# WeiZhang1988/YDORBSLAM

Measured on AMD Instinct MI355X. Metric: ORB extract+match Mkeypoints/sec, higher is better.
Workload: dtype u8

## Files before the change

ydorbslam_amd/csrc/extract_kernels.hip.h:

```cpp
#pragma once
#include <hip/hip_runtime.h>
#include <stdint.h>

#include "quadtree_core.h"
#include "quadtree_flat.h"

#pragma clang fp contract(off)

namespace ydorb {

constexpr int kPad = 19;
constexpr int kBorder = 16;
constexpr int kMaxLevels = 8;
constexpr int kTileMax = 72;
#ifndef QT_THREADS
#define QT_THREADS 512
#endif
constexpr int kQtThreads = QT_THREADS;

struct LevelDev {
  int w, h, pitch;
  int padOff;
  int blurOff, blurPitch;
  int cellBegin, nCells;
  int quota;
  int candOff;
  int kpOff;
  int tabOff;
  int nodeTabOff;
  float scale;
  float size;
};
struct PlanDev {
  int nLevels, nCellsTotal, cellCap, sumQuota;
  int maxX[16];
  unsigned nodeTabFrameStride;
  int blurTileBegin[kMaxLevels + 1];
  int borderBegin[kMaxLevels + 1];
  LevelDev lv[kMaxLevels];
};
#ifndef BLUR_TH
#define BLUR_TH 58
#endif
constexpr int kBlurTW = 64, kBlurTH = BLUR_TH;
struct CellDev {
  short level, x0, y0, x1, y1, pad0;
  int srcOff;
};

__device__ __forceinline__ int reflect101(int i, int n) {
  if (n == 1) return 0;
  while (i < 0 || i >= n) i = i < 0 ? -i : 2 * (n - 1) - i;
  return i;
}

typedef uint32_t __attribute__((aligned(1))) u32_unaligned;
typedef unsigned long long __attribute__((aligned(1))) u64_unaligned;

#ifndef PYR_ROWS
#define PYR_ROWS 8
#endif
constexpr int kPyrRows = PYR_ROWS;
__global__ __launch_bounds__(256) void k_pyr_level0(const uint8_t* __restrict__ img, int stride, size_t frameStride,
                                                    uint8_t* __restrict__ pyr, size_t pyrFrameStride, LevelDev L) {
  const int wx = blockIdx.x * 64 + (threadIdx.x & 63);
  const int yb = (blockIdx.y * 4 + __builtin_amdgcn_readfirstlane(threadIdx.x >> 6)) * kPyrRows;
  const int x0 = wx * 4 - kPad;
  if (x0 + 3 < 0 || x0 >= L.w) return;
  const uint8_t* src = img + (size_t)blockIdx.z * frameStride;
  uint8_t* dst = pyr + (size_t)blockIdx.z * pyrFrameStride + L.padOff + (size_t)kPad * L.pitch + wx * 4;
  const int xa = L.w >= 4 ? min(max(x0, 0), L.w - 4) : 0, sh = 8 * (x0 - xa);
  uint32_t v[kPyrRows];
// ... 294 lines not shown
    return;
  }
  {
    constexpr int COLS = PITCH == 48 ? 8 : 16, ROWS = 64 / COLS, NR = 6;
    const uint8_t* sub = pyr + (size_t)f * pyrFrameStride + c.srcOff;
    const int wpr = (tw + 7) >> 3, ty0 = lane / COLS, wd = lane % COLS;
    const bool colOk = wd < wpr;
    for (int tyb = 0; tyb < th; tyb += ROWS * NR) {
      unsigned long long r[NR];
#pragma unroll
      for (int k = 0; k < NR; k++) {
        const int ty = tyb + ty0 + ROWS * k;
        r[k] = (colOk && ty < th) ? *reinterpret_cast<const u64_unaligned*>(sub + (unsigned)(ty * pitch + 8 * wd)) : 0ull;
      }
#pragma unroll
      for (int k = 0; k < NR; k++) {
        const int ty = tyb + ty0 + ROWS * k;
        if (colOk && ty < th) *reinterpret_cast<unsigned long long*>(tile + ty * PITCH + 8 * wd) = r[k];
      }
    }
  }
  const int sw = bw + 2, sh = bh + 2;
  for (int i = lane; i < (sw * sh + 3) >> 2; i += 64) reinterpret_cast<uint32_t*>(score)[i] = 0;
  __builtin_amdgcn_wave_barrier();
  int n1 = 0;
  {
    const bool wide = bw > 32;
    const int bxl = wide ? lane : (lane & 31), byl = wide ? 0 : (lane >> 5), rowsPerIt = wide ? 1 : 2;
    const uint8_t* p = tile + (byl + 3) * PITCH + bxl + 3;
    unsigned ent = (unsigned)(byl << 6) | (unsigned)bxl;
    const uint16_t t16 = (uint16_t)thr;
    auto step = [&](uint16_t vmask) {
      const uint16_t v = p[0], a = p[3 * PITCH], b = p[-3 * PITCH], cc = p[3], d = p[-3];
      const uint16_t lo1 = min(a, b), hi1 = max(a, b), lo2 = min(cc, d), hi2 = max(cc, d);
      const uint16_t mx = max(lo1, lo2), mn = min(hi1, hi2);
      const uint16_t second = max(mx, mn), third = min(mn, mx);
      const uint16_t s1 = (uint16_t)((uint16_t)(v + t16) - second);
      const uint16_t s2 = (uint16_t)(third - (uint16_t)(v - t16));
      const bool keep = (int16_t)((uint16_t)(s1 | s2) & vmask) < 0;
      const unsigned long long m = __builtin_amdgcn_ballot_w64(keep);
      if (keep) list[n1 + wave_rank(m)] = (uint16_t)(ent | (s1 & 0x8000u) | ((s2 & 0x8000u) >> 1));
      n1 += __popcll(m);
      p += rowsPerIt * PITCH;
      ent += rowsPerIt * 64;
    };
    const bool colOk = bxl < bw;
    unsigned vmA = colOk ? 0xFFFFu : 0x7FFFu, vmF = colOk && byl == 0 ? 0xFFFFu : 0x7FFFu;
    asm volatile("" : "+v"(vmA), "+v"(vmF));
    const uint16_t vmAll = (uint16_t)vmA, vmFirst = (uint16_t)vmF;
    int by0 = 0;
    for (; by0 + rowsPerIt <= bh; by0 += rowsPerIt) step(vmAll);
    if (by0 < bh) step(vmFirst);
  }
  __builtin_amdgcn_wave_barrier();
  int n2 = 0;
  for (int base = 0; base < n1; base += 64) {
    const int j = base + lane;
    bool keep = false;
    unsigned ent = 0;
    if (j < n1) {
      ent = list[j];
      const int by = (ent >> 6) & 127, bx = ent & 63;
      const uint8_t* p = tile + (by + 3) * PITCH + bx + 3;
      const short v = (short)p[0];
      const bool dark = (ent & 0x4000u) != 0;
      const s16x2 sg = dark ? s16x2{1, 1} : s16x2{-1, -1};
      const s16x2 vs = s16x2{v, v} * sg, ng = -sg;
      s16x2 Pd[8];
      Pd[0] = s16x2{(short)p[3 * PITCH], (short)p[-3 * PITCH]} * ng + vs;
      Pd[1] = s16x2{(short)p[3 * PITCH + 1], (short)p[-3 * PITCH - 1]} * ng + vs;
      Pd[2] = s16x2{(short)p[2 * PITCH + 2], (short)p[-2 * PITCH - 2]} * ng + vs;
      Pd[3] = s16x2{(short)p[PITCH + 3], (short)p[-PITCH - 3]} * ng + vs;
      Pd[4] = s16x2{(short)p[3], (short)p[-3]} * ng + vs;
      Pd[5] = s16x2{(short)p[-PITCH + 3], (short)p[PITCH - 3]} * ng + vs;
      Pd[6] = s16x2{(short)p[-2 * PITCH + 2], (short)p[2 * PITCH - 2]} * ng + vs;
      Pd[7] = s16x2{(short)p[-3 * PITCH + 1], (short)p[3 * PITCH - 1]} * ng + vs;
      int best = fast_arc_best(Pd);
      if (__builtin_amdgcn_ballot_w64((ent & 0xC000u) == 0xC000u)) {
        if ((ent & 0xC000u) == 0xC000u) {
          s16x2 Nd[8];
#pragma unroll
          for (int k = 0; k < 8; k++) Nd[k] = -Pd[k];
          best = max(best, fast_arc_best(Nd));
        }
      }
      keep = best > thr;
      if (keep) score[(by + 1) * sw + bx + 1] = (uint8_t)(best - 1);
    }
    const unsigned long long m = __builtin_amdgcn_ballot_w64(keep);
    if (keep) list[n2 + wave_rank(m)] = (uint16_t)ent;
    n2 += __popcll(m);
  }
  __builtin_amdgcn_wave_barrier();
  int n3 = 0;
  uint32_t* dst = cellCand + slot * P.cellCap;
  for (int base = 0; base < n2; base += 64) {
    const int j = base + lane;
    bool keep = false;
    uint32_t rec = 0;
    if (j < n2) {
      const unsigned ent = list[j];
      const int by = (ent >> 6) & 127, bx = ent & 63;
      const uint8_t* q = &score[(by + 1) * sw + bx + 1];
      const uint16_t s = q[0];
      const uint16_t nb = max(max(max((uint16_t)q[-1], (uint16_t)q[1]), max((uint16_t)q[-sw - 1], (uint16_t)q[-sw])),
                              max(max((uint16_t)q[-sw + 1], (uint16_t)q[sw - 1]), max((uint16_t)q[sw], (uint16_t)q[sw + 1])));
      keep = s > nb;
      rec = qt_pack(c.x0 + 3 + bx - kBorder, c.y0 + 3 + by - kBorder, s);
    }
    const unsigned long long m = __builtin_amdgcn_ballot_w64(keep);
    const int pos = n3 + wave_rank(m);
    if (keep && pos < P.cellCap) dst[pos] = rec;
    n3 += __popcll(m);
  }
  if (lane == 0) cellCount[slot] = (uint32_t)min(n3, P.cellCap);
}


struct QtBlockCtx {
  unsigned* w32;
  unsigned long long* w64;
// ... 675 lines not shown
  const int ty = tileId / tilesX, tx = tileId - ty * tilesX;
  const int x0 = tx * TW, y0 = ty * TH;
  const uint8_t* padded = pyr + (size_t)f * pyrFrameStride + L.padOff;
  {
    const int r0 = threadIdx.x / SWW, wd = threadIdx.x - r0 * SWW;
    const int pcol = x0 + 16 + 4 * wd;
    const bool colOk = pcol < L.pitch;
    if (r0 < 14)
#pragma unroll
      for (int r = r0; r < SH; r += 14) {
        const int prow = min(y0 + r + kPad - 3, L.h + 2 * kPad - 1);
        src[r * SWW + wd] = colOk ? *reinterpret_cast<const uint32_t*>(padded + (size_t)prow * L.pitch + pcol) : 0u;
      }
  }
  __syncthreads();
  for (int task = threadIdx.x; task < (SH / 2) * (TW / 4); task += 256) {
    const int rp = task >> 4, g = task & 15;
    uint32_t o[2][4];
#pragma unroll
    for (int h = 0; h < 2; h++) {
      const int r = 2 * rp + h;
      const uint32_t w0 = src[r * SWW + g], w1 = src[r * SWW + g + 1], w2 = src[r * SWW + g + 2];
#pragma unroll
      for (int k = 0; k < 4; k++) {
        const uint32_t lo4 = k ? __builtin_amdgcn_alignbyte(w1, w0, k) : w0, hi4 = k ? __builtin_amdgcn_alignbyte(w2, w1, k) : w1;
        o[h][k] = __builtin_amdgcn_udot4(hi4, 0x00122230u, __builtin_amdgcn_udot4(lo4, 0x38302212u, 0u, false), false);
      }
    }
    *reinterpret_cast<uint4*>(&hb[rp * TW + g * 4]) =
        make_uint4(o[0][0] | (o[1][0] << 16), o[0][1] | (o[1][1] << 16), o[0][2] | (o[1][2] << 16), o[0][3] | (o[1][3] << 16));
  }
  __syncthreads();
  const int c4 = (threadIdx.x & 15) * 4;
#pragma unroll
  for (int r = threadIdx.x >> 4; r < TH; r += 16) {
    const int gy = y0 + r;
    if (!(gy < L.h && x0 + c4 < L.blurPitch)) continue;
    typedef unsigned short u16x2 __attribute__((ext_vector_type(2)));
    const bool odd = r & 1;
    const u16x2 k0 = odd ? u16x2{0, 18} : u16x2{18, 34}, k1 = odd ? u16x2{34, 48} : u16x2{48, 56};
    const u16x2 k2 = odd ? u16x2{56, 48} : u16x2{48, 34}, k3 = odd ? u16x2{34, 18} : u16x2{18, 0};
    const uint32_t* hp = &hb[(r >> 1) * TW + c4];
    const uint4 p0 = *reinterpret_cast<const uint4*>(hp), p1 = *reinterpret_cast<const uint4*>(hp + TW);
    const uint4 p2 = *reinterpret_cast<const uint4*>(hp + 2 * TW), p3 = *reinterpret_cast<const uint4*>(hp + 3 * TW);
    const uint32_t q0[4] = {p0.x, p0.y, p0.z, p0.w}, q1[4] = {p1.x, p1.y, p1.z, p1.w}, q2[4] = {p2.x, p2.y, p2.z, p2.w}, q3[4] = {p3.x, p3.y, p3.z, p3.w};
    uint32_t acc[4];
#pragma unroll
    for (int k = 0; k < 4; k++) {
      acc[k] = __builtin_amdgcn_udot2(__builtin_bit_cast(u16x2, q0[k]), k0, 32768u, false);
      acc[k] = __builtin_amdgcn_udot2(__builtin_bit_cast(u16x2, q1[k]), k1, acc[k], false);
      acc[k] = __builtin_amdgcn_udot2(__builtin_bit_cast(u16x2, q2[k]), k2, acc[k], false);
      acc[k] = __builtin_amdgcn_udot2(__builtin_bit_cast(u16x2, q3[k]), k3, acc[k], false);
    }
    const uint32_t out = (acc[0] >> 16) | ((acc[1] >> 16) << 8) | ((acc[2] >> 16) << 16) | ((acc[3] >> 16) << 24);
    *reinterpret_cast<uint32_t*>(blur + (size_t)f * blurFrameStride + L.blurOff + (size_t)gy * L.blurPitch + x0 + c4) = out;
  }
}

__device__ __forceinline__ float fast_atan2_deg(float y, float x) {
  const float p1 = 0.9997878412794807f * (float)(180 / 3.14159265358979323846);
  const float p3 = -0.3258083974640975f * (float)(180 / 3.14159265358979323846);
  const float p5 = 0.1555786518463281f * (float)(180 / 3.14159265358979323846);
  const float p7 = -0.04432655554792128f * (float)(180 / 3.14159265358979323846);
  const float eps = (float)2.2204460492503131e-16;
  const float ax = fabsf(x), ay = fabsf(y);
  float a, c, c2;
  if (ax >= ay) {
    c = __fdiv_rn(ay, __fadd_rn(ax, eps));
    c2 = __fmul_rn(c, c);
    a = __fmul_rn(__fadd_rn(__fmul_rn(__fadd_rn(__fmul_rn(__fadd_rn(__fmul_rn(p7, c2), p5), c2), p3), c2), p1), c);
  } else {
    c = __fdiv_rn(ax, __fadd_rn(ay, eps));
    c2 = __fmul_rn(c, c);
    a = __fsub_rn(90.f, __fmul_rn(__fadd_rn(__fmul_rn(__fadd_rn(__fmul_rn(__fadd_rn(__fmul_rn(p7, c2), p5), c2), p3), c2), p1), c));
// ... 107 lines not shown
  constexpr int kBias = 24;
  const uint8_t* bl = blur + (size_t)f * blurFrameStride + L.blurOff + (ptrdiff_t)(ky - kBias) * L.blurPitch + (kx - kBias);
  unsigned long long words[4];
#pragma unroll
  for (int t = 0; t < 4; t++) {
    const float4 pt = pat[t];
    const int r0 = __float2int_rn(__fadd_rn(__fmul_rn(pt.x, sinB), __fmul_rn(pt.y, cosA)));
    const int c0 = __float2int_rn(__fsub_rn(__fmul_rn(pt.x, cosA), __fmul_rn(pt.y, sinB)));
    const int r1 = __float2int_rn(__fadd_rn(__fmul_rn(pt.z, sinB), __fmul_rn(pt.w, cosA)));
    const int c1 = __float2int_rn(__fsub_rn(__fmul_rn(pt.z, cosA), __fmul_rn(pt.w, sinB)));
    const int t0 = bl[(unsigned)((r0 + kBias) * L.blurPitch + c0 + kBias)], t1 = bl[(unsigned)((r1 + kBias) * L.blurPitch + c1 + kBias)];
    words[t] = __ballot(t0 < t1);
  }
  if (lane < 4) {
    unsigned long long w = lane == 0 ? words[0] : lane == 1 ? words[1] : lane == 2 ? words[2] : words[3];
    reinterpret_cast<unsigned long long*>(desc + ((size_t)f * cap + outIdx) * 32)[lane] = w;
  }
  if (lane == 0) {
    YdKeyPointDev kp;
    kp.x = (float)kx;
    kp.y = (float)ky;
    if (level) { kp.x = __fmul_rn(kp.x, L.scale); kp.y = __fmul_rn(kp.y, L.scale); }
    kp.size = L.size;
    kp.angle = angle;
    kp.response = (float)qt_r(pk);
    kp.octave = level;
    kp.class_id = -1;
    kps[(size_t)f * cap + outIdx] = kp;
    lvlAngle[(size_t)f * P.sumQuota + slot] = angle;
  }
}


template <int KPW>
__global__ __launch_bounds__(256) void k_orient_describe_n(const uint8_t* __restrict__ pyr, size_t pyrFrameStride,
                                                           const uint8_t* __restrict__ blur, size_t blurFrameStride, PlanDev P,
                                                           const uint32_t* __restrict__ lvlKp, const int* __restrict__ lvlCount,
                                                           YdKeyPointDev* __restrict__ kps, uint8_t* __restrict__ desc, int cap,
                                                           int* __restrict__ nOut, float* __restrict__ lvlAngle) {
  const int lane = threadIdx.x & 63;
  int bx = blockIdx.x, f = blockIdx.y;
  if ((f | 7) < (int)gridDim.y) {
    bx = (f & 7) * (gridDim.x >> 3) + (blockIdx.x >> 3);
    f = (f & ~7) | (blockIdx.x & 7);
  }
  const int slot0 = (bx * 4 + __builtin_amdgcn_readfirstlane(threadIdx.x >> 6)) * KPW;
  if (slot0 >= P.sumQuota) return;
  float4 pat[4];
#pragma unroll
  for (int t = 0; t < 4; t++) pat[t] = reinterpret_cast<const float4*>(kPatternDev)[t * 64 + lane];
  int cnt[kMaxLevels], tot = 0;
#pragma unroll
  for (int l = 0; l < kMaxLevels; l++) { cnt[l] = l < P.nLevels ? lvlCount[f * kMaxLevels + l] : 0; tot += cnt[l]; }
  int level[KPW], outIdx[KPW];
  uint32_t pk[KPW];
  bool valid[KPW];
#pragma unroll
  for (int j = 0; j < KPW; j++) {
    const int slot = min(slot0 + j, P.sumQuota - 1);
    level[j] = 0;
#pragma unroll
    for (int l = 1; l < kMaxLevels; l++)
      if (l < P.nLevels && slot >= P.lv[l].kpOff) level[j] = l;
    pk[j] = __builtin_amdgcn_readfirstlane(lvlKp[(size_t)f * P.sumQuota + slot]);
  }
  if (slot0 == 0 && lane == 0) nOut[f] = min(tot, cap);
  bool any = false;
#pragma unroll
  for (int j = 0; j < KPW; j++) {
    int before = 0, mine = 0;
#pragma unroll
    for (int l = 0; l < kMaxLevels; l++) {
      if (l < level[j]) before += cnt[l];
      if (l == level[j]) mine = cnt[l];
    }
    const int k = slot0 + j - P.lv[level[j]].kpOff;
    outIdx[j] = before + k;
    valid[j] = slot0 + j < P.sumQuota && k < mine && outIdx[j] < cap;
    any = any || valid[j];
  }
  if (!any) return;
  int firstValid = 0;
#pragma unroll
  for (int j = KPW - 1; j >= 0; j--) if (valid[j]) firstValid = j;
#pragma unroll
  for (int j = 0; j < KPW; j++)
    if (!valid[j]) {
#pragma unroll
      for (int i = 0; i < KPW; i++) if (i == firstValid) { pk[j] = pk[i]; level[j] = level[i]; }
    }
  int kx[KPW], ky[KPW], pitch[KPW];
  const uint8_t* org[KPW];
#pragma unroll
  for (int j = 0; j < KPW; j++) {
    const LevelDev& L = P.lv[level[j]];
    kx[j] = qt_x(pk[j]) + kBorder; ky[j] = qt_y(pk[j]) + kBorder;
    pitch[j] = L.pitch;
    const uint8_t* roi = pyr + (size_t)f * pyrFrameStride + L.padOff + (size_t)kPad * L.pitch + kPad;
    org[j] = roi + (ptrdiff_t)(ky[j] - 15) * L.pitch + (kx[j] - 32);
  }
  const int u = lane - 32;
  unsigned narrow = 0;
#pragma unroll
  for (int v = 1; v <= 15; v++) narrow |= (unsigned)(P.maxX[v] == 0) << v;
  int m10[KPW], m01[KPW];
#pragma unroll
  for (int j = 0; j < KPW; j++) {
    m10[j] = 0; m01[j] = 0;
    if (u >= -15 && u <= 15) m10[j] = u * org[j][(unsigned)(15 * pitch[j] + lane)];
    if (lane >= 1 && lane <= 15 && ((narrow >> lane) & 1u)) {
      const int pos = org[j][(unsigned)((15 + lane) * pitch[j] + 32)], neg = org[j][(unsigned)((15 - lane) * pitch[j] + 32)];
      m01[j] = lane * (pos - neg);
    }
  }
#pragma unroll
  for (int v = 1; v <= 15; v++) {
    const int d = P.maxX[v];
    if (d > 0 && u >= -d && u <= d) {
#pragma unroll
      for (int j = 0; j < KPW; j++) {
        const int pos = org[j][(unsigned)((15 + v) * pitch[j] + lane)], neg = org[j][(unsigned)((15 - v) * pitch[j] + lane)];
        m01[j] += v * (pos - neg);
        m10[j] += u * (pos + neg);
      }
    }
  }
#pragma unroll
  for (int o = 32; o >= 1; o >>= 1) {
#pragma unroll
    for (int j = 0; j < KPW; j++) {
      m10[j] += __shfl_xor(m10[j], o, 64);
      m01[j] += __shfl_xor(m01[j], o, 64);
    }
  }
  constexpr int kBias = 24;
  float angle[KPW];
  int tA[KPW][4], tB[KPW][4];
#pragma unroll
  for (int j = 0; j < KPW; j++) {
    const LevelDev& L = P.lv[level[j]];
    angle[j] = fast_atan2_deg((float)m01[j], (float)m10[j]);
    const float rad = __fmul_rn(angle[j], (float)(3.14159265358979323846 / 180.0));
    float sinB, cosA;
    sincos_det(rad, &sinB, &cosA);
    const uint8_t* bl = blur + (size_t)f * blurFrameStride + L.blurOff + (ptrdiff_t)(ky[j] - kBias) * L.blurPitch + (kx[j] - kBias);
#pragma unroll
    for (int t = 0; t < 4; t++) {
      const float4 pt = pat[t];
      const int r0 = __float2int_rn(__fadd_rn(__fmul_rn(pt.x, sinB), __fmul_rn(pt.y, cosA)));
      const int c0 = __float2int_rn(__fsub_rn(__fmul_rn(pt.x, cosA), __fmul_rn(pt.y, sinB)));
      const int r1 = __float2int_rn(__fadd_rn(__fmul_rn(pt.z, sinB), __fmul_rn(pt.w, cosA)));
      const int c1 = __float2int_rn(__fsub_rn(__fmul_rn(pt.z, cosA), __fmul_rn(pt.w, sinB)));
      tA[j][t] = bl[(unsigned)((r0 + kBias) * L.blurPitch + c0 + kBias)];
      tB[j][t] = bl[(unsigned)((r1 + kBias) * L.blurPitch + c1 + kBias)];
    }
  }
#pragma unroll
  for (int j = 0; j < KPW; j++) {
    unsigned long long words[4];
#pragma unroll
    for (int t = 0; t < 4; t++) words[t] = __ballot(tA[j][t] < tB[j][t]);
    if (!valid[j]) continue;
    const LevelDev& L = P.lv[level[j]];
    if (lane < 4) {
      unsigned long long w = lane == 0 ? words[0] : lane == 1 ? words[1] : lane == 2 ? words[2] : words[3];
      reinterpret_cast<unsigned long long*>(desc + ((size_t)f * cap + outIdx[j]) * 32)[lane] = w;
    }
    if (lane == 0) {
      YdKeyPointDev kp;
      kp.x = (float)kx[j];
      kp.y = (float)ky[j];
      if (level[j]) { kp.x = __fmul_rn(kp.x, L.scale); kp.y = __fmul_rn(kp.y, L.scale); }
      kp.size = L.size;
      kp.angle = angle[j];
      kp.response = (float)qt_r(pk[j]);
      kp.octave = level[j];
      kp.class_id = -1;
      kps[(size_t)f * cap + outIdx[j]] = kp;
      lvlAngle[(size_t)f * P.sumQuota + slot0 + j] = angle[j];
    }
  }
}

}
```

ydorbslam_amd/csrc/orb_extractor.hip:

```cpp
#include <hip/hip_runtime.h>
#include <cstdlib>

#include <algorithm>
#include <cmath>
#include <cstdarg>
#include <cstdio>
#include <cstring>
#include <string>
#include <vector>

#include "../../include/ydorb/c_api.h"
#include "extract_kernels.hip.h"
#include "host_buffers.h"
#include "ydorb_host.h"

using namespace ydorb;

namespace {

inline int cvRoundF(float v) { return (int)lrintf(v); }
inline int cvFloorF(float v) { int i = (int)v; return i - (i > v); }
inline int alignUp(int v, int a) { return (v + a - 1) / a * a; }
inline size_t alignUpZ(size_t v, size_t a) { return (v + a - 1) / a * a; }

// ... 20 lines not shown
enum Stage { ST_PYR = 0, ST_FAST, ST_QT, ST_BLUR, ST_DESC, ST_COUNT };
const char* kStageNames[ST_COUNT] = {"pyramid", "fast_cells", "blur", "quadtree_after_blur", "orient_describe"};

}

struct ydorb_extractor {
  YdExtractorConfig cfg{};
  std::vector<float> sf, isf, sf2, isf2;
  std::vector<int> perLevel;
  int maxX[16]{};
  int sumQuota = 0;
  hipStream_t stream = nullptr;
  hipStream_t qtStream[kMaxLevels]{};
  hipEvent_t evFork = nullptr, evJoin[kMaxLevels]{};
  hipEvent_t evFast[kMaxLevels]{};
  int descKpw = 2;
  bool qtInline = false;
  int fastGroups = 1;
  HostPlan plan;
  bool planValid = false;
  int batchCap = 0;
  uint8_t *d_img = nullptr, *d_pyr = nullptr, *d_blur = nullptr;
  uint32_t *d_cellCount = nullptr, *d_cellCand = nullptr, *d_qtCand = nullptr, *d_qtKeys = nullptr, *d_lvlKp = nullptr;
  uint16_t* d_qtNode = nullptr;
  uint8_t* d_nodeScratch = nullptr;
  uint8_t* d_needPass = nullptr;
  int* d_passList = nullptr;
  int *d_lvlCount = nullptr, *d_status = nullptr, *d_nOut = nullptr;
  uint8_t* h_pyr = nullptr;
  size_t h_pyrBytes = 0;
  hipStream_t lastStream = nullptr;
  int *d_lvlMaxN = nullptr, *h_lvlMaxN = nullptr;
  float* d_lvlAngle = nullptr;
  CellDev* d_cells = nullptr;
  int* d_tabInt = nullptr;
  short* d_tabShort = nullptr;
  PyrPadEntry* d_padTab = nullptr;
  PyrColEntry* d_colTab = nullptr;
  int2* d_rowTab = nullptr;
  bool noFusedPads = false;
  YdKeyPointDev* d_kps = nullptr;
  uint8_t* d_desc = nullptr;
  size_t imgBytes = 0;
  uint8_t* h_img = nullptr;
  YdKeyPoint* h_kps = nullptr;
  uint8_t* h_desc = nullptr;
  int* h_nOut = nullptr;
  int* h_status = nullptr;
  int lastFrames = 0;
  bool profiling = false;
  bool profPending = false;
  bool forcePassQuadtree = false;
  hipEvent_t ev[ST_COUNT + 1]{};
  double stageMs[ST_COUNT]{};
  int stageCalls = 0;
};

namespace {

void freeBuffers(ydorb_extractor* e) {
  auto F = [](auto*& p) { if (p) { (void)hipFree(p); p = nullptr; } };
  F(e->d_img); F(e->d_pyr); F(e->d_blur); F(e->d_cellCount); F(e->d_cellCand); F(e->d_qtCand); F(e->d_qtKeys);
  F(e->d_lvlKp); F(e->d_qtNode); F(e->d_needPass); F(e->d_passList); F(e->d_nodeScratch); F(e->d_lvlCount); F(e->d_lvlMaxN); F(e->d_status); F(e->d_nOut); F(e->d_lvlAngle); F(e->d_cells);
  F(e->d_tabInt); F(e->d_tabShort); F(e->d_padTab); F(e->d_colTab); F(e->d_rowTab); F(e->d_kps); F(e->d_desc);
  auto H = [](auto*& p) { if (p) { (void)hipHostFree(p); p = nullptr; } };
  H(e->h_img); H(e->h_kps); H(e->h_desc); H(e->h_nOut); H(e->h_status); H(e->h_lvlMaxN); H(e->h_pyr);
  e->h_pyrBytes = 0;
  e->planValid = false;
}


static int qfItemsFor(long want) { return want <= 8L * kQfThreads ? 8 : want <= 16L * kQfThreads ? 16 : 32; }

void buildFusedLevel(HostPlan& P, int l) {
  const PlanDev& D = P.dev;
  const LevelDev& L = D.lv[l];
  HostPlan::FusedLevel& F = P.fused[l];
  F.on = false;
  if (L.w < 20 || L.h < 20) return;
  const int nd = (L.w + 2 * kPad + 3) >> 2;
  auto srcOf = [&](int p) { return p < kPad ? 2 * kPad - p : p < kPad + L.w ? -1 : p < L.w + 2 * kPad ? 2 * L.w + 2 * kPad - 2 - p : -2; };
  int shift = -1;
  for (int sft = 0; sft < 64 && shift < 0; sft++) {
    bool ok = true;
    for (int c = 0; c < nd && ok; c++)
      for (int j = 0; j < 4; j++) {
        const int sp = srcOf(4 * c + j);
        if (sp >= 0 && ((sp >> 2) + sft) >> 6 != (c + sft) >> 6) ok = false;
      }
    if (ok) shift = sft;
  }
  if (shift < 0) return;
  std::vector<PyrColEntry> col;
  if (l > 0) {
    const LevelDev& Lp = D.lv[l - 1];
    const int* xofs = P.tabInt.data() + P.tab[l].xofs;
// ... 21 lines not shown
      if (dA < 0 || d == dA) dA = d;
      else dB = d;
    }
    PyrPadEntry pe{};
    pe.laneA4 = 4u * (unsigned)(((dA < 0 ? c : dA) + shift) & 63);
    pe.laneB4 = 4u * (unsigned)(((dB < 0 ? c : dB) + shift) & 63);
    pe.selM = 0; pe.selF = 0;
    for (int j = 0; j < 4; j++) {
      const int sp = srcOf(4 * c + j);
      uint32_t m = 0x0c, f;
      if (sp == -1) f = (uint32_t)j;
      else if (sp == -2) f = 0x0c;
      else { m = (uint32_t)(sp & 3) + ((sp >> 2) == dA ? 4u : 0u); f = 4u + (uint32_t)j; }
      pe.selM |= m << (8 * j);
      pe.selF |= f << (8 * j);
    }
    P.padTab.push_back(pe);
  }
  if (l > 0) {
    F.colOff = (int)P.colTab.size();
    P.colTab.insert(P.colTab.end(), col.begin(), col.end());
    F.rowOff = (int)P.rowTab.size();
    const int* yofs = P.tabInt.data() + P.tab[l].yofs;
    const short* beta = P.tabShort.data() + P.tab[l].beta;
    const int rows = alignUp(L.h, 4 * kPyrRowsF);
    for (int y = 0; y < rows; y++) {
      const int dy = std::min(y, L.h - 1);
      P.rowTab.push_back(make_int2(yofs[dy], (int)((uint32_t)(uint16_t)beta[2 * dy] | ((uint32_t)(uint16_t)beta[2 * dy + 1] << 16))));
    }
  }
  F.on = true;
}

int buildPlan(ydorb_extractor* e, int w, int h, HostPlan& P) {
  P = HostPlan();
  P.w = w; P.h = h;
  PlanDev& D = P.dev;
  D.nLevels = e->cfg.n_levels;
  for (int v = 0; v < 16; v++) D.maxX[v] = e->maxX[v];
  size_t padOff = 0, blurOff = 0;
  int kpOff = 0, candOff = 0, maxCellDim = 0;
  for (int l = 0; l < D.nLevels; l++) {
    LevelDev& L = D.lv[l];
    L.w = cvRoundF((float)w * e->isf[l]);
    L.h = cvRoundF((float)h * e->isf[l]);
    if (L.w < 1 || L.h < 1 || L.w > 4000 || L.h > 4000) {
      set_error("level %d size %dx%d out of the supported range (1..4000)", l, L.w, L.h);
      return YDORB_ERR_UNSUPPORTED;
    }
    L.pitch = alignUp(L.w + 2 * kPad, 64);
    L.padOff = (int)padOff;
    padOff += alignUpZ((size_t)(L.h + 2 * kPad) * L.pitch, 256);
    L.blurPitch = alignUp(L.w, 64);
    L.blurOff = (int)blurOff;
    blurOff += alignUpZ((size_t)L.h * L.blurPitch, 256);
    L.quota = e->perLevel[l];
    L.kpOff = kpOff;
    kpOff += L.quota;
    L.scale = e->sf[l];
    L.size = (float)(int)(31 * e->sf[l]);
    L.cellBegin = (int)P.cells.size();
    const int minB = kBorder, maxBX = L.w - kBorder, maxBY = L.h - kBorder;
    const float width = (float)(maxBX - minB), height = (float)(maxBY - minB);
    const int colsNum = (int)(width / 30.0f), rowsNum = (int)(height / 30.0f);
    if (colsNum > 0 && rowsNum > 0) {
      const int cellW = (int)ceilf(width / colsNum), cellH = (int)ceilf(height / rowsNum);
      maxCellDim = std::max(maxCellDim, std::max(cellW, cellH));
      P.levelCellDim[l] = std::max(cellW, cellH);
      for (int i = 0; i < rowsNum; i++) {
        const float iniY = (float)(minB + i * cellH);
        float maxY = iniY + cellH + 6;
        if (iniY >= maxBY - 3) continue;
        if (maxY > maxBY) maxY = (float)maxBY;
        for (int j = 0; j < colsNum; j++) {
          const float iniX = (float)(minB + j * cellW);
          float maxX = iniX + cellW + 6;
          if (iniX >= maxBX - 6) continue;
          if (maxX > maxBX) maxX = (float)maxBX;
          CellDev c{};
          c.level = (short)l;
          c.x0 = (short)iniX; c.y0 = (short)iniY; c.x1 = (short)maxX; c.y1 = (short)maxY;
          c.srcOff = L.padOff + (kPad + c.y0) * L.pitch + kPad + c.x0;
          P.cells.push_back(c);
        }
      }
    }
// ... 77 lines not shown
  }
  P.qtPassLds = std::max<size_t>(P.qtPassLds, 1024);
  return YDORB_OK;
}

int ensurePlan(ydorb_extractor* e, int w, int h, int nFrames) {
  if (e->planValid && e->plan.w == w && e->plan.h == h && nFrames <= e->batchCap) return YDORB_OK;
  HIPCHK(hipStreamSynchronize(e->stream));
  HostPlan P;
  int rc = buildPlan(e, w, h, P);
  if (rc) return rc;
  freeBuffers(e);
  const int B = std::max(nFrames, std::max(1, e->cfg.max_batch));
  e->plan = P;
  e->batchCap = B;
  e->imgBytes = (size_t)w * h;
  const PlanDev& D = P.dev;
  HIPCHK(hipMalloc(&e->d_img, e->imgBytes * B));
  HIPCHK(hipMalloc(&e->d_pyr, P.pyrFrameStride * B));
  HIPCHK(hipMemsetAsync(e->d_pyr, 0, P.pyrFrameStride * B, e->stream));
  HIPCHK(hipMalloc(&e->d_blur, P.blurFrameStride * B));
  HIPCHK(hipMalloc(&e->d_cellCount, sizeof(uint32_t) * D.nCellsTotal * B));
  HIPCHK(hipMalloc(&e->d_cellCand, sizeof(uint32_t) * (size_t)D.nCellsTotal * D.cellCap * B));
  HIPCHK(hipMalloc(&e->d_qtCand, sizeof(uint32_t) * 2 * P.qtFrameStride * B));
  HIPCHK(hipMalloc(&e->d_qtNode, sizeof(uint16_t) * 2 * P.qtFrameStride * B));
  if (D.nodeTabFrameStride) HIPCHK(hipMalloc(&e->d_nodeScratch, (size_t)D.nodeTabFrameStride * B));
  HIPCHK(hipMalloc(&e->d_needPass, (size_t)kMaxLevels * B));
  HIPCHK(hipMemsetAsync(e->d_needPass, 0, (size_t)kMaxLevels * B, e->stream));
  HIPCHK(hipMalloc(&e->d_passList, sizeof(int) * ((size_t)kMaxLevels * B + 1)));
  HIPCHK(hipMemsetAsync(e->d_passList, 0, sizeof(int), e->stream));

  HIPCHK(hipMalloc(&e->d_lvlKp, sizeof(uint32_t) * (size_t)D.sumQuota * B));
  HIPCHK(hipMalloc(&e->d_lvlAngle, sizeof(float) * (size_t)D.sumQuota * B));
  HIPCHK(hipMalloc(&e->d_lvlCount, sizeof(int) * kMaxLevels * B));
  HIPCHK(hipMalloc(&e->d_lvlMaxN, sizeof(int) * (kMaxLevels + 1)));
  HIPCHK(hipMemsetAsync(e->d_lvlMaxN, 0, sizeof(int) * (kMaxLevels + 1), e->stream));
  HIPCHK(hipHostMalloc(&e->h_lvlMaxN, sizeof(int) * (kMaxLevels + 1)));
  memset(e->h_lvlMaxN, 0, sizeof(int) * (kMaxLevels + 1));
  HIPCHK(hipMalloc(&e->d_status, sizeof(int)));
  HIPCHK(hipMalloc(&e->d_nOut, sizeof(int) * B));
  HIPCHK(hipMalloc(&e->d_cells, sizeof(CellDev) * std::max<size_t>(P.cells.size(), 1)));
  HIPCHK(hipMalloc(&e->d_tabInt, sizeof(int) * std::max<size_t>(P.tabInt.size(), 1)));
  HIPCHK(hipMalloc(&e->d_tabShort, sizeof(short) * std::max<size_t>(P.tabShort.size(), 1)));
  HIPCHK(hipMalloc(&e->d_kps, sizeof(YdKeyPointDev) * (size_t)D.sumQuota * B));
  HIPCHK(hipMalloc(&e->d_desc, (size_t)32 * D.sumQuota * B));
  HIPCHK(hipHostMalloc(&e->h_img, e->imgBytes * B));
  HIPCHK(hipHostMalloc(&e->h_kps, sizeof(YdKeyPoint) * (size_t)D.sumQuota * B));
  HIPCHK(hipHostMalloc(&e->h_desc, (size_t)32 * D.sumQuota * B));
  HIPCHK(hipHostMalloc(&e->h_nOut, sizeof(int) * B));
  HIPCHK(hipHostMalloc(&e->h_status, sizeof(int)));
  if (!P.cells.empty()) HIPCHK(hipMemcpyAsync(e->d_cells, P.cells.data(), sizeof(CellDev) * P.cells.size(), hipMemcpyHostToDevice, e->stream));
  if (!P.tabInt.empty()) HIPCHK(hipMemcpyAsync(e->d_tabInt, P.tabInt.data(), sizeof(int) * P.tabInt.size(), hipMemcpyHostToDevice, e->stream));
  if (!P.tabShort.empty()) HIPCHK(hipMemcpyAsync(e->d_tabShort, P.tabShort.data(), sizeof(short) * P.tabShort.size(), hipMemcpyHostToDevice, e->stream));
  HIPCHK(hipMalloc(&e->d_padTab, sizeof(PyrPadEntry) * std::max<size_t>(P.padTab.size(), 1)));
  HIPCHK(hipMalloc(&e->d_colTab, sizeof(PyrColEntry) * std::max<size_t>(P.colTab.size(), 1)));
  HIPCHK(hipMalloc(&e->d_rowTab, sizeof(int2) * std::max<size_t>(P.rowTab.size(), 1)));
  if (!P.padTab.empty()) HIPCHK(hipMemcpyAsync(e->d_padTab, P.padTab.data(), sizeof(PyrPadEntry) * P.padTab.size(), hipMemcpyHostToDevice, e->stream));
  if (!P.colTab.empty()) HIPCHK(hipMemcpyAsync(e->d_colTab, P.colTab.data(), sizeof(PyrColEntry) * P.colTab.size(), hipMemcpyHostToDevice, e->stream));
  if (!P.rowTab.empty()) HIPCHK(hipMemcpyAsync(e->d_rowTab, P.rowTab.data(), sizeof(int2) * P.rowTab.size(), hipMemcpyHostToDevice, e->stream));
  HIPCHK(hipMemsetAsync(e->d_status, 0, sizeof(int), e->stream));
  HIPCHK(hipStreamSynchronize(e->stream));
  if (std::max(P.qtLdsMax, P.qtPassLds) > 48 * 1024)
  {
    HIPCHK(hipFuncSetAttribute(reinterpret_cast<const void*>(k_quadtree), hipFuncAttributeMaxDynamicSharedMemorySize, (int)std::max(P.qtLdsMax, P.qtPassLds)));
    HIPCHK(hipFuncSetAttribute(reinterpret_cast<const void*>(k_quadtree_list), hipFuncAttributeMaxDynamicSharedMemorySize, (int)std::max(P.qtLdsMax, P.qtPassLds)));
  }
// ... 218 lines not shown
  if (const char* v = getenv("YDORB_DESC_KPW")) e->descKpw = atoi(v) == 1 ? 1 : atoi(v) == 4 ? 4 : 2;
  e->cfg.min_fast_thr = cfg->ini_fast_thr;
  const int L = cfg->n_levels;
  const float s = cfg->scale_factor;
  int per = (int)round(cfg->n_features * (1 - 1.0 / s) / (1.0 - pow(1.0 / s, L)));
  int sum = 0;
  for (int i = 0; i < L; i++) {
    e->sf.push_back((float)pow(s, i));
    e->sf2.push_back((float)pow(s, 2 * i));
    e->isf.push_back((float)pow(s, -i));
    e->isf2.push_back((float)pow(s, -2 * i));
    if (i < L - 1) {
      e->perLevel.push_back(per);
      sum += per;
      per = (int)round((float)per / s);
    } else {
      e->perLevel.push_back(std::max(cfg->n_features - sum, 0));
    }
  }
  e->sumQuota = 0;
  for (int q : e->perLevel) e->sumQuota += q;
  {
    const int half = 15;
    std::vector<int> mx(half + 1, 0);
    const int maxY = (int)floor(half * sqrt(2.0) / 2.0 + 1.0), minY = (int)ceil(half * sqrt(2.0) / 2.0);
    for (int v = 0; v <= maxY; v++) mx.push_back((int)round(sqrt((double)half * half + (double)v * v)));
    for (int v = half, i = 0; v >= minY; v--) {
      while (mx[i] == mx[i + 1]) i++;
      mx[v] = i;
      i++;
    }
    for (int v = 0; v < 16; v++) e->maxX[v] = mx[v];
  }
  if (hipStreamCreateWithFlags(&e->stream, hipStreamNonBlocking) != hipSuccess) {
    set_error("hipStreamCreate failed");
    delete e;
    return YDORB_ERR_HIP;
  }
  for (auto& ev : e->ev) (void)hipEventCreate(&ev);
  (void)hipEventCreateWithFlags(&e->evFork, hipEventDisableTiming);
  for (int l = 0; l < kMaxLevels; l++) {
    const char* qtEnv = getenv("YDORB_QT_STREAMS");
    e->qtInline = (qtEnv && atoi(qtEnv) == 0) || (cfg->flags & YDORB_EXTRACTOR_SINGLE_STREAM);
    const int nQt = std::max(1, std::min(qtEnv ? atoi(qtEnv) : (cfg->max_batch <= 8 ? (int)kMaxLevels : 2), (int)kMaxLevels));
    if (l < nQt) (void)hipStreamCreateWithFlags(&e->qtStream[l], hipStreamNonBlocking);
    else e->qtStream[l] = e->qtStream[l % nQt];
    (void)hipEventCreateWithFlags(&e->evJoin[l], hipEventDisableTiming);
    (void)hipEventCreateWithFlags(&e->evFast[l], hipEventDisableTiming);
  }
  {
    const char* g = getenv("YDORB_FAST_GROUPS");
    e->fastGroups = std::max(1, std::min(g ? atoi(g) : (cfg->max_batch <= 8 ? 1 : 2), (int)kMaxLevels));
  }
  *out = e;
  return YDORB_OK;
}

void ydorb_extractor_destroy(ydorb_extractor_t* e) {
  if (!e) return;
  (void)hipSetDevice(e->cfg.device);
  if (e->stream) (void)hipStreamSynchronize(e->stream);
  freeBuffers(e);
  for (auto& ev : e->ev) if (ev) (void)hipEventDestroy(ev);
  for (int l = 0; l < kMaxLevels; l++) {
    if (e->qtStream[l]) {
      bool shared = false;
// ... 243 lines not shown
```

Baseline: 181.9.

## Compute orientation moments with packed-byte sdot4 lane table and DPP reductions

Replaces the per-row byte-gather loop for the intensity-centroid moments with a precomputed table. Each lane loads 4-byte pixel groups over three steps and accumulates m10/m01 with signed dot4, using XOR 0x80 biasing and zero-sum weights to cancel the offset. The shuffle-xor butterfly is replaced by DPP reductions, and atan2/sincos now runs once per wave, with lane j serving keypoint j. The change also uses mul24 addressing plus a new pitch limit check, packed f32x2 pattern rotation, a single-lane 2x uint4 descriptor store, and blur kernel constants hoisted out of the row loop.

```diff
diff --git a/ydorbslam_amd/csrc/extract_kernels.hip.h b/ydorbslam_amd/csrc/extract_kernels.hip.h
--- a/ydorbslam_amd/csrc/extract_kernels.hip.h
+++ b/ydorbslam_amd/csrc/extract_kernels.hip.h
@@ -12,6 +12,8 @@
 constexpr int kPad = 19;
 constexpr int kBorder = 16;
 constexpr int kMaxLevels = 8;
+constexpr int kMomentSteps = 3;
+constexpr int kMaxPitch24 = 1 << 18;
 constexpr int kTileMax = 72;
 #ifndef QT_THREADS
 #define QT_THREADS 512
@@ -38,6 +40,7 @@
   int blurTileBegin[kMaxLevels + 1];
   int borderBegin[kMaxLevels + 1];
   LevelDev lv[kMaxLevels];
+  const uint4* momentTab;
 };
 #ifndef BLUR_TH
 #define BLUR_TH 58
@@ -1194,14 +1197,17 @@
   }
   __syncthreads();
   const int c4 = (threadIdx.x & 15) * 4;
+  typedef unsigned short u16x2 __attribute__((ext_vector_type(2)));
+  const bool odd = (threadIdx.x >> 4) & 1;
+  uint32_t kw0 = odd ? 0x00120000u : 0x00220012u, kw1 = odd ? 0x00300022u : 0x00380030u;
+  uint32_t kw2 = odd ? 0x00300038u : 0x00220030u, kw3 = odd ? 0x00120022u : 0x00000012u;
+  asm volatile("" : "+v"(kw0), "+v"(kw1), "+v"(kw2), "+v"(kw3));
+  const u16x2 k0 = __builtin_bit_cast(u16x2, kw0), k1 = __builtin_bit_cast(u16x2, kw1);
+  const u16x2 k2 = __builtin_bit_cast(u16x2, kw2), k3 = __builtin_bit_cast(u16x2, kw3);
 #pragma unroll
   for (int r = threadIdx.x >> 4; r < TH; r += 16) {
     const int gy = y0 + r;
     if (!(gy < L.h && x0 + c4 < L.blurPitch)) continue;
-    typedef unsigned short u16x2 __attribute__((ext_vector_type(2)));
-    const bool odd = r & 1;
-    const u16x2 k0 = odd ? u16x2{0, 18} : u16x2{18, 34}, k1 = odd ? u16x2{34, 48} : u16x2{48, 56};
-    const u16x2 k2 = odd ? u16x2{56, 48} : u16x2{48, 34}, k3 = odd ? u16x2{34, 18} : u16x2{18, 0};
     const uint32_t* hp = &hb[(r >> 1) * TW + c4];
     const uint4 p0 = *reinterpret_cast<const uint4*>(hp), p1 = *reinterpret_cast<const uint4*>(hp + TW);
     const uint4 p2 = *reinterpret_cast<const uint4*>(hp + 2 * TW), p3 = *reinterpret_cast<const uint4*>(hp + 3 * TW);
@@ -1375,12 +1381,23 @@
 }
 
 
+__device__ __forceinline__ int wave_sum_lane63(int x) {
+  x += __builtin_amdgcn_update_dpp(0, x, 0xB1, 0xf, 0xf, false);
+  x += __builtin_amdgcn_update_dpp(0, x, 0x4E, 0xf, 0xf, false);
+  x += __builtin_amdgcn_update_dpp(0, x, 0x141, 0xf, 0xf, false);
+  x += __builtin_amdgcn_update_dpp(0, x, 0x140, 0xf, 0xf, false);
+  x += __builtin_amdgcn_update_dpp(0, x, 0x142, 0xa, 0xf, false);
+  x += __builtin_amdgcn_update_dpp(0, x, 0x143, 0xc, 0xf, false);
+  return x;
+}
+
 template <int KPW>
 __global__ __launch_bounds__(256) void k_orient_describe_n(const uint8_t* __restrict__ pyr, size_t pyrFrameStride,
                                                            const uint8_t* __restrict__ blur, size_t blurFrameStride, PlanDev P,
                                                            const uint32_t* __restrict__ lvlKp, const int* __restrict__ lvlCount,
                                                            YdKeyPointDev* __restrict__ kps, uint8_t* __restrict__ desc, int cap,
                                                            int* __restrict__ nOut, float* __restrict__ lvlAngle) {
+  typedef float f32x2 __attribute__((ext_vector_type(2)));
   const int lane = threadIdx.x & 63;
   int bx = blockIdx.x, f = blockIdx.y;
   if ((f | 7) < (int)gridDim.y) {
@@ -1392,6 +1409,9 @@
   float4 pat[4];
 #pragma unroll
   for (int t = 0; t < 4; t++) pat[t] = reinterpret_cast<const float4*>(kPatternDev)[t * 64 + lane];
+  uint4 mt[kMomentSteps];
+#pragma unroll
+  for (int st = 0; st < kMomentSteps; st++) mt[st] = P.momentTab[st * 64 + lane];
   int cnt[kMaxLevels], tot = 0;
 #pragma unroll
   for (int l = 0; l < kMaxLevels; l++) { cnt[l] = l < P.nLevels ? lvlCount[f * kMaxLevels + l] : 0; tot += cnt[l]; }
@@ -1433,69 +1453,65 @@
       for (int i = 0; i < KPW; i++) if (i == firstValid) { pk[j] = pk[i]; level[j] = level[i]; }
     }
   int kx[KPW], ky[KPW], pitch[KPW];
-  const uint8_t* org[KPW];
+  size_t org[KPW];
 #pragma unroll
   for (int j = 0; j < KPW; j++) {
     const LevelDev& L = P.lv[level[j]];
     kx[j] = qt_x(pk[j]) + kBorder; ky[j] = qt_y(pk[j]) + kBorder;
     pitch[j] = L.pitch;
-    const uint8_t* roi = pyr + (size_t)f * pyrFrameStride + L.padOff + (size_t)kPad * L.pitch + kPad;
-    org[j] = roi + (ptrdiff_t)(ky[j] - 15) * L.pitch + (kx[j] - 32);
-  }
-  const int u = lane - 32;
-  unsigned narrow = 0;
-#pragma unroll
-  for (int v = 1; v <= 15; v++) narrow |= (unsigned)(P.maxX[v] == 0) << v;
+    org[j] = (size_t)f * pyrFrameStride + L.padOff + (size_t)(kPad + ky[j] - 15) * L.pitch + (kPad + kx[j] - 32);
+    asm volatile("" : "+s"(org[j]));
+  }
   int m10[KPW], m01[KPW];
 #pragma unroll
+  for (int j = 0; j < KPW; j++) { m10[j] = 0; m01[j] = 0; }
+  {
+    uint32_t px[kMomentSteps][KPW];
+#pragma unroll
+    for (int st = 0; st < kMomentSteps; st++) {
+      const unsigned row = mt[st].x & 0xffu, col = mt[st].x >> 8;
+#pragma unroll
+      for (int j = 0; j < KPW; j++) px[st][j] = *reinterpret_cast<const u32_unaligned*>(pyr + org[j] + (__umul24(row, pitch[j]) + col));
+    }
+#pragma unroll
+    for (int st = 0; st < kMomentSteps; st++)
+#pragma unroll
+      for (int j = 0; j < KPW; j++) {
+        const int x = (int)(px[st][j] ^ 0x80808080u);
+        m10[j] = __builtin_amdgcn_sdot4(x, (int)mt[st].y, m10[j], false);
+        m01[j] = __builtin_amdgcn_sdot4(x, (int)mt[st].z, m01[j], false);
+      }
+  }
+  int a01 = 0, a10 = 0;
+#pragma unroll
   for (int j = 0; j < KPW; j++) {
-    m10[j] = 0; m01[j] = 0;
-    if (u >= -15 && u <= 15) m10[j] = u * org[j][(unsigned)(15 * pitch[j] + lane)];
-    if (lane >= 1 && lane <= 15 && ((narrow >> lane) & 1u)) {
-      const int pos = org[j][(unsigned)((15 + lane) * pitch[j] + 32)], neg = org[j][(unsigned)((15 - lane) * pitch[j] + 32)];
-      m01[j] = lane * (pos - neg);
-    }
-  }
-#pragma unroll
-  for (int v = 1; v <= 15; v++) {
-    const int d = P.maxX[v];
-    if (d > 0 && u >= -d && u <= d) {
-#pragma unroll
-      for (int j = 0; j < KPW; j++) {
-        const int pos = org[j][(unsigned)((15 + v) * pitch[j] + lane)], neg = org[j][(unsigned)((15 - v) * pitch[j] + lane)];
-        m01[j] += v * (pos - neg);
-        m10[j] += u * (pos + neg);
-      }
-    }
-  }
-#pragma unroll
-  for (int o = 32; o >= 1; o >>= 1) {
-#pragma unroll
-    for (int j = 0; j < KPW; j++) {
-      m10[j] += __shfl_xor(m10[j], o, 64);
-      m01[j] += __shfl_xor(m01[j], o, 64);
-    }
-  }
+    const int s01 = __builtin_amdgcn_readlane(wave_sum_lane63(m01[j]), 63), s10 = __builtin_amdgcn_readlane(wave_sum_lane63(m10[j]), 63);
+    if (j == 0 || lane == j) { a01 = s01; a10 = s10; }
+  }
+  const float angleV = fast_atan2_deg((float)a01, (float)a10);
+  float sinV, cosV;
+  sincos_det(__fmul_rn(angleV, (float)(3.14159265358979323846 / 180.0)), &sinV, &cosV);
   constexpr int kBias = 24;
   float angle[KPW];
   int tA[KPW][4], tB[KPW][4];
 #pragma unroll
   for (int j = 0; j < KPW; j++) {
     const LevelDev& L = P.lv[level[j]];
-    angle[j] = fast_atan2_deg((float)m01[j], (float)m10[j]);
-    const float rad = __fmul_rn(angle[j], (float)(3.14159265358979323846 / 180.0));
-    float sinB, cosA;
-    sincos_det(rad, &sinB, &cosA);
-    const uint8_t* bl = blur + (size_t)f * blurFrameStride + L.blurOff + (ptrdiff_t)(ky[j] - kBias) * L.blurPitch + (kx[j] - kBias);
+    angle[j] = __builtin_bit_cast(float, __builtin_amdgcn_readlane(__builtin_bit_cast(int, angleV), j));
+    const float sinB = __builtin_bit_cast(float, __builtin_amdgcn_readlane(__builtin_bit_cast(int, sinV), j));
+    const float cosA = __builtin_bit_cast(float, __builtin_amdgcn_readlane(__builtin_bit_cast(int, cosV), j));
+    const f32x2 sc = {sinB, cosA}, cs = {cosA, -sinB};
+    const int bp = L.blurPitch;
+    const uint8_t* bl = blur + (size_t)f * blurFrameStride + L.blurOff + (ptrdiff_t)(ky[j] - kBias) * bp + (kx[j] - kBias);
+    const int biasOff = kBias * bp + kBias;
 #pragma unroll
     for (int t = 0; t < 4; t++) {
       const float4 pt = pat[t];
-      const int r0 = __float2int_rn(__fadd_rn(__fmul_rn(pt.x, sinB), __fmul_rn(pt.y, cosA)));
-      const int c0 = __float2int_rn(__fsub_rn(__fmul_rn(pt.x, cosA), __fmul_rn(pt.y, sinB)));
-      const int r1 = __float2int_rn(__fadd_rn(__fmul_rn(pt.z, sinB), __fmul_rn(pt.w, cosA)));
-      const int c1 = __float2int_rn(__fsub_rn(__fmul_rn(pt.z, cosA), __fmul_rn(pt.w, sinB)));
-      tA[j][t] = bl[(unsigned)((r0 + kBias) * L.blurPitch + c0 + kBias)];
-      tB[j][t] = bl[(unsigned)((r1 + kBias) * L.blurPitch + c1 + kBias)];
+      const f32x2 rc0 = f32x2{pt.x, pt.x} * sc + f32x2{pt.y, pt.y} * cs;
+      const f32x2 rc1 = f32x2{pt.z, pt.z} * sc + f32x2{pt.w, pt.w} * cs;
+      const int r0 = __float2int_rn(rc0.x), c0 = __float2int_rn(rc0.y), r1 = __float2int_rn(rc1.x), c1 = __float2int_rn(rc1.y);
+      tA[j][t] = bl[(unsigned)(__mul24(r0, bp) + c0 + biasOff)];
+      tB[j][t] = bl[(unsigned)(__mul24(r1, bp) + c1 + biasOff)];
     }
   }
 #pragma unroll
@@ -1505,11 +1521,10 @@
     for (int t = 0; t < 4; t++) words[t] = __ballot(tA[j][t] < tB[j][t]);
     if (!valid[j]) continue;
     const LevelDev& L = P.lv[level[j]];
-    if (lane < 4) {
-      unsigned long long w = lane == 0 ? words[0] : lane == 1 ? words[1] : lane == 2 ? words[2] : words[3];
-      reinterpret_cast<unsigned long long*>(desc + ((size_t)f * cap + outIdx[j]) * 32)[lane] = w;
-    }
     if (lane == 0) {
+      uint4* d = reinterpret_cast<uint4*>(desc + ((size_t)f * cap + outIdx[j]) * 32);
+      d[0] = make_uint4((uint32_t)words[0], (uint32_t)(words[0] >> 32), (uint32_t)words[1], (uint32_t)(words[1] >> 32));
+      d[1] = make_uint4((uint32_t)words[2], (uint32_t)(words[2] >> 32), (uint32_t)words[3], (uint32_t)(words[3] >> 32));
       YdKeyPointDev kp;
       kp.x = (float)kx[j];
       kp.y = (float)ky[j];
diff --git a/ydorbslam_amd/csrc/orb_extractor.hip b/ydorbslam_amd/csrc/orb_extractor.hip
--- a/ydorbslam_amd/csrc/orb_extractor.hip
+++ b/ydorbslam_amd/csrc/orb_extractor.hip
@@ -76,6 +76,8 @@
   hipStream_t lastStream = nullptr;
   int *d_lvlMaxN = nullptr, *h_lvlMaxN = nullptr;
   float* d_lvlAngle = nullptr;
+  std::vector<uint4> momentTab;
+  uint4* d_momentTab = nullptr;
   CellDev* d_cells = nullptr;
   int* d_tabInt = nullptr;
   short* d_tabShort = nullptr;
@@ -105,7 +107,7 @@
 void freeBuffers(ydorb_extractor* e) {
   auto F = [](auto*& p) { if (p) { (void)hipFree(p); p = nullptr; } };
   F(e->d_img); F(e->d_pyr); F(e->d_blur); F(e->d_cellCount); F(e->d_cellCand); F(e->d_qtCand); F(e->d_qtKeys);
-  F(e->d_lvlKp); F(e->d_qtNode); F(e->d_needPass); F(e->d_passList); F(e->d_nodeScratch); F(e->d_lvlCount); F(e->d_lvlMaxN); F(e->d_status); F(e->d_nOut); F(e->d_lvlAngle); F(e->d_cells);
+  F(e->d_lvlKp); F(e->d_qtNode); F(e->d_needPass); F(e->d_passList); F(e->d_nodeScratch); F(e->d_lvlCount); F(e->d_lvlMaxN); F(e->d_status); F(e->d_nOut); F(e->d_lvlAngle); F(e->d_momentTab); F(e->d_cells);
   F(e->d_tabInt); F(e->d_tabShort); F(e->d_padTab); F(e->d_colTab); F(e->d_rowTab); F(e->d_kps); F(e->d_desc);
   auto H = [](auto*& p) { if (p) { (void)hipHostFree(p); p = nullptr; } };
   H(e->h_img); H(e->h_kps); H(e->h_desc); H(e->h_nOut); H(e->h_status); H(e->h_lvlMaxN); H(e->h_pyr);
@@ -193,6 +195,26 @@
   F.on = true;
 }
 
+bool buildMomentTab(const int* maxX, std::vector<uint4>& tab) {
+  tab.clear();
+  long sumU = 0, sumV = 0;
+  for (int v = -15; v <= 15; v++) {
+    const int d = v == 0 ? 15 : maxX[v < 0 ? -v : v];
+    for (int c = -d; c <= d; c += 4) {
+      uint32_t wu = 0, wv = 0;
+      for (int b = 0; b < 4 && c + b <= d; b++) {
+        wu |= (uint32_t)(uint8_t)(int8_t)(c + b) << (8 * b);
+        wv |= (uint32_t)(uint8_t)(int8_t)v << (8 * b);
+        sumU += c + b; sumV += v;
+      }
+      tab.push_back(make_uint4((uint32_t)(15 + v) | (uint32_t)(32 + c) << 8, wu, wv, 0u));
+    }
+  }
+  if (sumU != 0 || sumV != 0 || tab.size() > (size_t)kMomentSteps * 64) return false;
+  tab.resize((size_t)kMomentSteps * 64, make_uint4(15u | 32u << 8, 0u, 0u, 0u));
+  return true;
+}
+
 int buildPlan(ydorb_extractor* e, int w, int h, HostPlan& P) {
   P = HostPlan();
   P.w = w; P.h = h;
@@ -213,6 +235,10 @@
     L.padOff = (int)padOff;
     padOff += alignUpZ((size_t)(L.h + 2 * kPad) * L.pitch, 256);
     L.blurPitch = alignUp(L.w, 64);
+    if (L.pitch >= kMaxPitch24 || L.blurPitch >= kMaxPitch24) {
+      set_error("level %d row pitch %d is beyond the 24-bit address arithmetic of the descriptor kernel (< %d)", l, L.pitch, kMaxPitch24);
+      return YDORB_ERR_CAPACITY;
+    }
     L.blurOff = (int)blurOff;
     blurOff += alignUpZ((size_t)L.h * L.blurPitch, 256);
     L.quota = e->perLevel[l];
@@ -356,6 +382,9 @@
 
   HIPCHK(hipMalloc(&e->d_lvlKp, sizeof(uint32_t) * (size_t)D.sumQuota * B));
   HIPCHK(hipMalloc(&e->d_lvlAngle, sizeof(float) * (size_t)D.sumQuota * B));
+  HIPCHK(hipMalloc(&e->d_momentTab, sizeof(uint4) * e->momentTab.size()));
+  HIPCHK(hipMemcpyAsync(e->d_momentTab, e->momentTab.data(), sizeof(uint4) * e->momentTab.size(), hipMemcpyHostToDevice, e->stream));
+  e->plan.dev.momentTab = e->d_momentTab;
   HIPCHK(hipMalloc(&e->d_lvlCount, sizeof(int) * kMaxLevels * B));
   HIPCHK(hipMalloc(&e->d_lvlMaxN, sizeof(int) * (kMaxLevels + 1)));
   HIPCHK(hipMemsetAsync(e->d_lvlMaxN, 0, sizeof(int) * (kMaxLevels + 1), e->stream));
@@ -640,6 +669,11 @@
     }
     for (int v = 0; v < 16; v++) e->maxX[v] = mx[v];
   }
+  if (!buildMomentTab(e->maxX, e->momentTab)) {
+    set_error("the orientation patch does not fit the descriptor kernel's lane table");
+    delete e;
+    return YDORB_ERR_UNSUPPORTED;
+  }
   if (hipStreamCreateWithFlags(&e->stream, hipStreamNonBlocking) != hipSuccess) {
     set_error("hipStreamCreate failed");
     delete e;
```

Measured after the change: 181.8, median of 2. No clear change (-0.1%).

## Defer second-polarity FAST arc checks to a list tail and simplify prefilter

Applied to the files above, without the earlier changes.

The second-stage FAST check no longer runs the opposite-polarity arc test inside a divergent branch. When a candidate flagged both bright and dark fails its first test, it is appended to the end of the candidate list with its flags cleared. A later wave iteration then re-tests it in the other polarity, falling back to in-place evaluation on the last chunk or when list capacity is tight. The 4-point prefilter is also rewritten with fewer min/max operations, using a different order statistic of the cross pixels. The aim is to cut wave divergence and ALU work, at the cost of extra list traffic, more complex bookkeeping, and possibly a different set of candidates passing the prefilter.

```diff
diff --git a/ydorbslam_amd/csrc/extract_kernels.hip.h b/ydorbslam_amd/csrc/extract_kernels.hip.h
--- a/ydorbslam_amd/csrc/extract_kernels.hip.h
+++ b/ydorbslam_amd/csrc/extract_kernels.hip.h
@@ -398,14 +398,12 @@
     const uint16_t t16 = (uint16_t)thr;
     auto step = [&](uint16_t vmask) {
       const uint16_t v = p[0], a = p[3 * PITCH], b = p[-3 * PITCH], cc = p[3], d = p[-3];
-      const uint16_t lo1 = min(a, b), hi1 = max(a, b), lo2 = min(cc, d), hi2 = max(cc, d);
-      const uint16_t mx = max(lo1, lo2), mn = min(hi1, hi2);
-      const uint16_t second = max(mx, mn), third = min(mn, mx);
-      const uint16_t s1 = (uint16_t)((uint16_t)(v + t16) - second);
-      const uint16_t s2 = (uint16_t)(third - (uint16_t)(v - t16));
+      const uint16_t mn = min(max(a, b), max(cc, d)), mx = max(min(a, b), min(cc, d));
+      const uint16_t s1 = (uint16_t)((uint16_t)(v + t16) - mn);
+      const uint16_t s2 = (uint16_t)(mx - (uint16_t)(v - t16));
       const bool keep = (int16_t)((uint16_t)(s1 | s2) & vmask) < 0;
       const unsigned long long m = __builtin_amdgcn_ballot_w64(keep);
-      if (keep) list[n1 + wave_rank(m)] = (uint16_t)(ent | (s1 & 0x8000u) | ((s2 & 0x8000u) >> 1));
+      if (keep) list[n1 + wave_rank(m)] = (uint16_t)(ent | (s1 & 0x8000u) | (s2 & 0x4000u));
       n1 += __popcll(m);
       p += rowsPerIt * PITCH;
       ent += rowsPerIt * 64;
@@ -419,10 +417,12 @@
     if (by0 < bh) step(vmFirst);
   }
   __builtin_amdgcn_wave_barrier();
+  const int listCap = lds.listBytes >> 1;
   int n2 = 0;
   for (int base = 0; base < n1; base += 64) {
     const int j = base + lane;
-    bool keep = false;
+    const bool inPlace = base + 64 >= n1 || n1 + 64 > listCap;
+    bool keep = false, defer = false;
     unsigned ent = 0;
     if (j < n1) {
       ent = list[j];
@@ -442,17 +442,22 @@
       Pd[6] = s16x2{(short)p[-2 * PITCH + 2], (short)p[2 * PITCH - 2]} * ng + vs;
       Pd[7] = s16x2{(short)p[-3 * PITCH + 1], (short)p[3 * PITCH - 1]} * ng + vs;
       int best = fast_arc_best(Pd);
-      if (__builtin_amdgcn_ballot_w64((ent & 0xC000u) == 0xC000u)) {
-        if ((ent & 0xC000u) == 0xC000u) {
-          s16x2 Nd[8];
-#pragma unroll
-          for (int k = 0; k < 8; k++) Nd[k] = -Pd[k];
-          best = max(best, fast_arc_best(Nd));
-        }
+      const unsigned flags = ent & 0xC000u;
+      const bool again = flags == 0xC000u && best <= thr;
+      if (again && inPlace) {
+        s16x2 Nd[8];
+#pragma unroll
+        for (int k = 0; k < 8; k++) Nd[k] = -Pd[k];
+        best = fast_arc_best(Nd);
       }
-      keep = best > thr;
-      if (keep) score[(by + 1) * sw + bx + 1] = (uint8_t)(best - 1);
-    }
+      const bool pass = best > thr;
+      if (pass) score[(by + 1) * sw + bx + 1] = (uint8_t)(best - 1);
+      defer = again && !inPlace;
+      keep = (pass && flags != 0) || defer;
+    }
+    const unsigned long long md = __builtin_amdgcn_ballot_w64(defer);
+    if (defer) list[n1 + wave_rank(md)] = (uint16_t)(ent & 0x3FFFu);
+    n1 += __popcll(md);
     const unsigned long long m = __builtin_amdgcn_ballot_w64(keep);
     if (keep) list[n2 + wave_rank(m)] = (uint16_t)ent;
     n2 += __popcll(m);
```

Result: no change. 182.8 before, 182.6 after (-0.1%).
